# SarodYatawatta/smart-calibration

Hardware: AMD Instinct MI355X
Metric: env-steps/sec (whole node), elastic-net SAC (higher is better)
Workload: dtype fp32; 1 GPU; model=elasticnet-sac, N=20, M=20, input_dims=420, global_batch=64, replay=1024, reward_scale=20, prioritized=False, parallelism=dp1

## Files before the change

### setup.py

```python

import os
from pathlib import Path

from setuptools import setup

os.environ.setdefault("PYTORCH_ROCM_ARCH", "gfx950")

from torch.utils.cpp_extension import BuildExtension, CUDAExtension

ROOT = Path(__file__).resolve().parent
CSRC = ROOT / "smartcal_amd" / "ops" / "csrc"

sources = [str(CSRC / f) for f in [
    "bindings.hip",
    "fused_linear.hip",
    "gemm_f32.hip",
    "elementwise.hip",
    "enet_solver.hip",
    "als_sweep.hip",
    "conv2d.hip",
    "per.hip",
    "fused_linear_bf16.hip",
    "attention.hip",
    "cgemm.hip",
    "coherency.hip",
    "shapelet.hip",
    "beam.hip",
    "dft_image.hip",
    "hessianres.hip",
    "two_loop.hip",
    "gather_sum.hip",
]]

# ... 17 lines not shown
```

### smartcal_amd/envs/enet.py

```python

from __future__ import annotations

from typing import Optional

import numpy as np
import torch

from .. import gymapi
from ..gymapi import spaces
from ..ops import enet as enet_ops
from ..utils.device import default_device

LOW = 1e-3
HIGH = 1e-1


class ENetEnv(gymapi.Env):

    metadata = {"render.modes": ["human"]}

    def __init__(self, M: int = 5, N: int = 15, provide_hint: bool = False,
                 device: Optional[torch.device] = None):
        super().__init__()
        self.K = 2
# ... 20 lines not shown
        self._sample_problem()

    def _sample_problem(self):
        dev = self.device
        A = torch.randn(self.N, self.M, dtype=torch.float32, device=dev)
        self.A = A / torch.norm(A)
        self.Mo = int(torch.randint(3, self.M, (1,)).item())
        z0 = torch.randn(self.Mo, dtype=torch.float32, device=dev)
        self.x0 = torch.zeros(self.M, dtype=torch.float32, device=dev)
        self.x0[np.random.randint(0, self.M, self.Mo)] = z0
        self.y0 = self.A @ self.x0

    def _observe_y(self):
        n = torch.randn(self.N, dtype=torch.float32, device=self.device)
        self.y = self.y0 + self.SNR * torch.norm(self.y0) / torch.norm(n) * n

    def reset(self):
        self._sample_problem()
        self.hint = None
        self.rho = LOW * torch.ones(self.K, dtype=torch.float32)
        observation = {
            "A": self.A.reshape(-1),
            "eig": torch.zeros(self.N, dtype=torch.float32,
                               device=self.device),
        }
        return observation

    def step(self, action, keepnoise: bool = False):
        done = False
        if not torch.is_tensor(action):
            action = torch.as_tensor(np.asarray(action).reshape(-1),
                                     dtype=torch.float32)
        action = action.detach().reshape(-1)
        action = torch.nan_to_num(action, nan=0.0, posinf=1.0, neginf=-1.0)

        if self.device.type == "cuda" and action.device == self.device:
            scaled = action * (HIGH - LOW) / 2 + (HIGH + LOW) / 2
            penalty = -0.1 * ((scaled < LOW).sum() + (scaled > HIGH).sum())
            rho = scaled.clamp(LOW, HIGH)
            self.rho = rho
            if not keepnoise or self.y is None:
                self._observe_y()
            x, EE, reward = enet_ops.solve_and_influence_device(
                self.A, self.y, rho, penalty.to(torch.float32))
            self.x = x
            EE = torch.nan_to_num(EE, nan=0.0, posinf=1e6, neginf=-1e6)
            reward = torch.nan_to_num(reward, nan=-100.0, posinf=1e6,
                                      neginf=-1e6)
            observation = {"A": self.A.reshape(-1), "eig": EE}
            info: dict = {}
            if self.provide_hint:
                if self.hint is None:
                    self.hint = self.get_hint()
                return observation, reward, done, self.hint, info
            return observation, reward, done, info

        action = action.to("cpu", torch.float32)
        self.rho = action * (HIGH - LOW) / 2 + (HIGH + LOW) / 2
        penalty = 0.0
        for ci in range(self.K):
            if self.rho[ci] < LOW:
                self.rho[ci] = LOW
                penalty += -0.1
            if self.rho[ci] > HIGH:
                self.rho[ci] = HIGH
                penalty += -0.1

        if not keepnoise or self.y is None:
            self._observe_y()

        x, EE, reward = enet_ops.solve_and_influence(
# ... 65 lines not shown
                if mse < best[1]:
                    best = ((l1, l2), mse)
        hint_ = np.array(best[0], dtype=np.float64)
        return (hint_ - (HIGH + LOW) / 2) / ((HIGH - LOW) / 2)

    def close(self):
        pass


def obs_to_state(observation) -> torch.Tensor:
    if not isinstance(observation, dict):
        if torch.is_tensor(observation):
            return observation.reshape(-1).to(torch.float32)
        return torch.as_tensor(np.asarray(observation),
                               dtype=torch.float32).reshape(-1)
    eig = observation["eig"]
    A = observation["A"]
    if not torch.is_tensor(eig):
        eig = torch.as_tensor(eig, dtype=torch.float32)
    if not torch.is_tensor(A):
        A = torch.as_tensor(A, dtype=torch.float32)
    return torch.cat((eig.reshape(-1), A.reshape(-1).to(eig.device)))

try:
    from sklearn.base import BaseEstimator as _SKBase
except Exception:
    _SKBase = object


class SKEnet(_SKBase):
# ... 23 lines not shown
```

### smartcal_amd/envs/vec_enet.py

```python

from __future__ import annotations

from typing import Optional

import numpy as np
import torch

from ..ops import enet as enet_ops
from ..utils.device import default_device
from .enet import HIGH, LOW


class VecENetEnv:

    def __init__(self, E: int, M: int = 5, N: int = 15,
                 reward_clamp: Optional[float] = None,
                 device: Optional[torch.device] = None):
        self.E = int(E)
        self.M = int(M)
        self.N = int(N)
        self.K = 2
        self.reward_clamp = reward_clamp
        self.device = device if device is not None else default_device()
        self.SNR = 0.1
# ... 24 lines not shown
        self._sample_problems()
        self.y = None
        return {"A": self.A.reshape(self.E, -1),
                "eig": torch.zeros(self.E, self.N, dtype=torch.float32,
                                   device=self.device)}

    def step(self, actions, keepnoise: bool = False):
        if torch.is_tensor(actions):
            a = actions.detach().to(dtype=torch.float32) \
                .reshape(self.E, self.K)
        else:
            a = torch.as_tensor(np.asarray(actions), dtype=torch.float32) \
                .reshape(self.E, self.K)
        if a.device != self.device:
            a = a.to(self.device)
        a = torch.nan_to_num(a.detach(), nan=0.0, posinf=1.0, neginf=-1.0)
        scaled = a * (HIGH - LOW) / 2 + (HIGH + LOW) / 2
        penalty = -0.1 * ((scaled < LOW).sum(1)
                          + (scaled > HIGH).sum(1)).to(torch.float32)
        rho = scaled.clamp(LOW, HIGH)
        self.rho = rho
        if not keepnoise or self.y is None:
            self._observe_y()
        x, EE, reward = enet_ops.solve_and_influence_batch(
            self.A, self.y, rho, penalty)
        self.x = x
        EE = torch.nan_to_num(EE, nan=0.0, posinf=1e6, neginf=-1e6)
        reward = torch.nan_to_num(reward, nan=-100.0, posinf=1e6,
                                  neginf=-1e6)
        if self.reward_clamp is not None:
            reward = reward.clamp(-self.reward_clamp, self.reward_clamp)
        obs = {"A": self.A.reshape(self.E, -1), "eig": EE}
        done = torch.zeros(self.E, dtype=torch.bool, device=self.device)
        return obs, reward, done, {}

    def solution_error(self) -> torch.Tensor:
        return ((self.x0 - self.x).norm(dim=1)
                / self.x0.norm(dim=1).clamp(min=1e-12))
```

### smartcal_amd/ops/csrc/bindings.hip

```cpp

#include <ATen/hip/HIPContext.h>
#include <c10/hip/HIPStream.h>
#include <torch/extension.h>

#include <algorithm>
#include <tuple>

#include "common.h"

#define HMAX 7

extern "C" __global__ void fused_linear_fwd_kernel(
    const float*, const float*, const float*, const float*, const float*,
    float*, float*, float*, int, int, int, int, int);
extern "C" __global__ void ln_act_bwd_kernel(const float*, const float*,
                                             const float*, const float*,
                                             const float*, float*, float*,
                                             float*, int, int, int, int,
                                             int);
extern "C" __global__ void gemm_f32_nn_kernel(const float*, const float*,
                                              float*, int, int, int);
extern "C" __global__ void gemm_f32_tn_kernel(const float*, const float*,
                                              float*, float*, int, int, int,
                                              int);
// ... 16 lines not shown
extern "C" __global__ void conv2d_k5s2_fwd_kernel(
    const float*, const float*, const float*, float*, int, int, int, int,
    int, int, int);
extern "C" __global__ void conv2d_k5s2_dx_kernel(
    const float*, const float*, float*, int, int, int, int, int, int, int);
extern "C" __global__ void conv2d_k5s2_dw_kernel(
    const float*, const float*, float*, float*, int, int, int, int, int,
    int, int);
struct c32b { float x, y; };
extern "C" __global__ void als_sweep_kernel(
    const c32b*, const c32b*, const c32b*, const int*, const int*,
    const int*, c32b*, c32b*, int, int, int, int, int, int);
extern "C" __global__ void enet_influence_kernel(
    const float*, const float*, const float*, const float*, const float*,
    const int*, const float*, const float*, float*, float*, int, int, int);
extern "C" __global__ void per_sample_kernel(const float*, const float*,
                                             long*, float*, float*, int, int,
                                             float);
extern "C" __global__ void fused_linear_bf16_fwd_kernel(
    const float*, const float*, const float*, const float*, const float*,
    float*, float*, float*, int, int, int, int, int);
extern "C" __global__ void gemm_bf16_nn_kernel(const float*, const float*,
                                               float*, int, int, int);
extern "C" __global__ void gemm_bf16_tn_kernel(const float*, const float*,
                                               float*, int, int, int, int);
extern "C" __global__ void attn_fwd_kernel(const float*, const float*,
                                           const float*, float*, float*,
                                           int, int, int);
extern "C" __global__ void attn_bwd_kernel(const float*, const float*,
                                           const float*, const float*,
// ... 607 lines not shown
                     (int)history);
  return {x, Y, S, nh};
}

std::tuple<at::Tensor, at::Tensor> enet_influence(
    const at::Tensor& A, const at::Tensor& y, const at::Tensor& x,
    const at::Tensor& Y, const at::Tensor& S, const at::Tensor& nh,
    const at::Tensor& penalty, const at::Tensor& rho) {
  check_f32(A, "A");
  check_f32(rho, "rho");
  const int E = A.size(0), N = A.size(1), M = A.size(2);
  TORCH_CHECK(N <= 32 && M <= 32, "enet influence supports N,M <= 32");
  TORCH_CHECK(rho.numel() == 2 * E, "rho must be (E, 2)");
  auto EE = at::empty({E, N}, A.options());
  auto reward = at::empty({E}, A.options());
  const int lds_floats = N * M + M * N + N * N + 2 * HMAX * M + HMAX * N + N
                         + M + N + HMAX;
  hipLaunchKernelGGL(enet_influence_kernel, dim3(E), dim3(64),
                     lds_floats * sizeof(float), stream(),
                     A.data_ptr<float>(), y.data_ptr<float>(),
                     x.data_ptr<float>(), Y.data_ptr<float>(),
                     S.data_ptr<float>(), nh.data_ptr<int>(),
                     penalty.data_ptr<float>(), rho.data_ptr<float>(),
                     EE.data_ptr<float>(), reward.data_ptr<float>(),
                     E, N, M);
  return {EE, reward};
}

#define PER_LDS_MAX_N 32768
#define PER_MAX_B 4096

std::tuple<at::Tensor, at::Tensor, at::Tensor> per_sample(
    const at::Tensor& priorities, const at::Tensor& u, double beta) {
  check_f32(priorities, "priorities");
  check_f32(u, "u");
  const int n = priorities.numel();
  const int B = u.numel();
  TORCH_CHECK(n >= 1 && n <= PER_LDS_MAX_N,
              "per_sample: n must be in [1, 32768]");
  TORCH_CHECK(B >= 1 && B <= PER_MAX_B, "per_sample: B must be in [1, 4096]");
  auto idx = at::empty({B}, priorities.options().dtype(at::kLong));
// ... 392 lines not shown
  m.def("fused_linear_bwd_dz_into", &fused_linear_bwd_dz_into);
  m.def("mlp_chain_fwd", &mlp_chain_fwd, py::arg("x"), py::arg("Ws"),
        py::arg("bs"), py::arg("gammas"), py::arg("betas"), py::arg("acts"),
        py::arg("bf16") = false, py::arg("save") = true);
  m.def("critic_fwd", &critic_fwd, py::arg("state"), py::arg("action"),
        py::arg("Ws"), py::arg("bs"), py::arg("gammas"), py::arg("betas"),
        py::arg("acts"), py::arg("save") = true);
  m.def("als_sweep", &als_sweep);
  m.def("conv2d_k5s2_fwd", &conv2d_k5s2_fwd);
  m.def("conv2d_k5s2_bwd", &conv2d_k5s2_bwd);
  m.def("tanh_gauss_fwd", &tanh_gauss_fwd);
  m.def("tanh_gauss_bwd", &tanh_gauss_bwd);
  m.def("fused_adam", &fused_adam);
  m.def("enet_lbfgs_solve", &enet_lbfgs_solve);
  m.def("enet_influence", &enet_influence);
  m.def("per_sample", &per_sample);
  m.def("per_update", &per_update);
  m.def("fused_linear_bf16_fwd", &fused_linear_bf16_fwd);
  m.def("mfma_gemm_nn_bf16", &mfma_gemm_nn_bf16);
  m.def("mfma_gemm_tn_bias_into_bf16", &mfma_gemm_tn_bias_into_bf16);
  m.def("attn_fwd", &attn_fwd);
  m.def("attn_bwd", &attn_bwd);
  m.def("cgemm_nn_bcast", &cgemm_nn_bcast);
  m.def("coherency_predict", &coherency_predict);
  m.def("shapelet_predict", &shapelet_predict, py::arg("C"),
        py::arg("uvw_scaled"), py::arg("hdr"), py::arg("coff"),
        py::arg("coef"), py::arg("clk"), py::arg("soff"), py::arg("fdelta"),
        py::arg("E") = py::none(), py::arg("p") = py::none(),
        py::arg("q") = py::none(), py::arg("sbase") = 0);
  m.def("station_beam", &station_beam);
// ... 9 lines not shown
```

### smartcal_amd/ops/csrc/enet_solver.hip

```cpp

#include "common.h"

#define HMAX 7
#define TOL_GRAD 1e-7f
#define TOL_CHANGE 1e-9f
#define NMAX 32

struct LdsLayout {
  float* __restrict__ A;
  float* __restrict__ y;
  float* __restrict__ x;
  float* __restrict__ g;
  float* __restrict__ gprev;
  float* __restrict__ d;
  float* __restrict__ x0;
  float* __restrict__ r;
  float* __restrict__ S;
  float* __restrict__ Yh;
  float* __restrict__ bg0;
  float* __restrict__ bg1;
  float* __restrict__ ro;
  float* __restrict__ al;
  float* __restrict__ xprev;
};
// ... 200 lines not shown
  }

  if (!done) {
    t = br_t[low];
    f_new = br_f[low];
    if (lane < M) {
      L.g[lane] = br_g[low][lane];
      float xd = t * L.d[lane];
      L.x[lane] = L.x0[lane] + (isfinite(xd) ? xd : 0.f);
    }
  }
  *t_io = t;
  return f_new;
}

extern "C" __global__ __launch_bounds__(64) void enet_lbfgs_solve_kernel(
    const float* __restrict__ Ag,
    const float* __restrict__ yg,
    const float* __restrict__ rhog,
    float* __restrict__ xg,
    float* __restrict__ Yg,
    float* __restrict__ Sg,
    int* __restrict__ nhistg,
    int E, int N, int M, int epochs, int max_iter, int history) {
  extern __shared__ float smem[];
  const int env = blockIdx.x;
  const int lane = threadIdx.x;
  if (history > HMAX) history = HMAX;

  LdsLayout L;
  float* p = smem;
  L.A = p; p += N * M;
  L.y = p; p += N;
  L.x = p; p += M;
  L.g = p; p += M;
  L.gprev = p; p += M;
  L.d = p; p += M;
  L.x0 = p; p += M;
  L.r = p; p += N;
  L.S = p; p += HMAX * M;
  L.Yh = p; p += HMAX * M;
  L.bg0 = p; p += M;
  L.bg1 = p; p += M;
  L.ro = p; p += HMAX;
  L.al = p; p += HMAX;
  L.xprev = p; p += M;

  for (int i = lane; i < N * M; i += WAVE) L.A[i] = Ag[(long)env * N * M + i];
  __builtin_amdgcn_s_barrier();
  RegA Ar;
#pragma unroll
  for (int j = 0; j < 32; ++j)
    Ar.row[j] = (lane < N && j < M) ? L.A[lane * M + j] : 0.f;
#pragma unroll
  for (int i = 0; i < 32; ++i)
    Ar.col[i] = (lane < M && i < N) ? L.A[i * M + lane] : 0.f;
  if (lane < N) L.y[lane] = yg[(long)env * N + lane];
  if (lane < M) {
    L.x[lane] = 0.f;
    L.d[lane] = 0.f;
    L.gprev[lane] = 0.f;
  }
  const float rho1 = rhog[env * 2 + 0];
  const float rho2 = rhog[env * 2 + 1];

  int nhist = 0;
  int n_iter = 0;
  float t = 1.f, H_diag = 1.f, prev_loss = 0.f;
  float prev_epoch_loss = 1e30f;
  if (lane < M) L.xprev[lane] = 1e30f;

  for (int epoch = 0; epoch < epochs; ++epoch) {
    float loss = eval_loss_grad(L, Ar, N, M, rho1, rho2);
    if (fabsf(loss - prev_epoch_loss) <= 3e-7f * fmaxf(1.f, fabsf(loss)))
      break;
    prev_epoch_loss = loss;
    {
      float dx = (lane < M) ? fabsf(L.x[lane] - L.xprev[lane]) : 0.f;
      float dmax = wave_max(dx);
// ... 73 lines not shown
      loss = strong_wolfe(L, Ar, N, M, rho1, rho2, loss, gtd, &t);
      if (!isfinite(loss)) {
        if (lane < M) L.x[lane] = L.x0[lane];
        loss = eval_loss_grad(L, Ar, N, M, rho1, rho2);
        outer_done = true;
        break;
      }

      if (lds_absmax(L.g, M) <= TOL_GRAD) { outer_done = true; break; }
      float step_max = lds_absmax(L.d, M) * fabsf(t);
      if (step_max <= TOL_CHANGE) break;
      if (fabsf(loss - prev_loss) < TOL_CHANGE) break;
    }
    if (outer_done) break;
  }

  if (lane < M) xg[(long)env * M + lane] = L.x[lane];
  for (int h = 0; h < HMAX; ++h) {
    if (lane < M) {
      float yv = (h < nhist) ? L.Yh[h * M + lane] : 0.f;
      float sv = (h < nhist) ? L.S[h * M + lane] : 0.f;
      Yg[((long)env * HMAX + h) * M + lane] = yv;
      Sg[((long)env * HMAX + h) * M + lane] = sv;
    }
  }
  if (lane == 0) nhistg[env] = nhist;
}

extern "C" __global__ __launch_bounds__(64) void enet_influence_kernel(
    const float* __restrict__ Ag,
    const float* __restrict__ yg,
    const float* __restrict__ xg,
    const float* __restrict__ Yg,
    const float* __restrict__ Sg,
    const int* __restrict__ nhistg,
    const float* __restrict__ peng,
    const float* __restrict__ rhog,
    float* __restrict__ EEg,
    float* __restrict__ rewardg,
    int E, int N, int M) {
  extern __shared__ float smem[];
  const int env = blockIdx.x;
  const int lane = threadIdx.x;
  const int nh = nhistg[env];

  float* p = smem;
  float* A = p; p += N * M;
  float* Q = p; p += M * N;
  float* B = p; p += N * N;
  float* Sv = p; p += HMAX * M;
  float* Yv = p; p += HMAX * M;
  float* alv = p; p += HMAX * N;
  float* ev = p; p += N;
  float* xs = p; p += M;
  float* ys_ = p; p += N;
  float* ro = p; p += HMAX;

  for (int i = lane; i < N * M; i += WAVE) A[i] = Ag[(long)env * N * M + i];
  for (int i = lane; i < HMAX * M; i += WAVE) {
    Sv[i] = Sg[(long)env * HMAX * M + i];
    Yv[i] = Yg[(long)env * HMAX * M + i];
  }
  if (lane < M) xs[lane] = xg[(long)env * M + lane];
  if (lane < N) ys_[lane] = yg[(long)env * N + lane];

  __builtin_amdgcn_s_barrier();
  float qc[32];
#pragma unroll
  for (int m = 0; m < 32; ++m)
    qc[m] = (lane < N && m < M) ? -2.f * A[lane * M + m] : 0.f;

  const float rho1f = rhog[env * 2];
  const float lo = fmaxf(1e-6f, rho1f);
  const float hi = 8.f * (1.f + rho1f) * (1.f + rho1f);
  float ys = 1.f, yy = 1.f;
  for (int i = 0; i < nh; ++i) {
    float ysi = lds_dot(&Yv[i * M], &Sv[i * M], M);
    float ssi = lds_dot(&Sv[i * M], &Sv[i * M], M);
    float yyi = lds_dot(&Yv[i * M], &Yv[i * M], M);
    float r = (ysi > lo * ssi && yyi < hi * ssi) ? 1.f / ysi : 0.f;
    if (lane == 0) ro[i] = r;
    if (r != 0.f) {
      ys = ysi;
      yy = yyi;
    }
  }
  __builtin_amdgcn_s_barrier();
// ... 90 lines not shown
  const float ee_floor = 1.f - 1.f / fmaxf(rho1f, 1e-6f);
  if (lane < N) ev[lane] = fmaxf(B[lane * N + lane] + 1.f, ee_floor);

  for (int phase = 0; phase < N; ++phase) {
    int start = phase & 1;
    int i0 = start + 2 * lane;
    float a0 = 0.f, a1 = 0.f;
    bool act = (i0 + 1 < N);
    if (act) { a0 = ev[i0]; a1 = ev[i0 + 1]; }
    if (act && a0 > a1) {
      ev[i0] = a1;
      ev[i0 + 1] = a0;
    }
  }

  if (lane < N) EEg[(long)env * N + lane] = ev[lane];

  float ri = 0.f, yl = 0.f;
  if (lane < N) {
    float ax = 0.f;
    for (int m = 0; m < M; ++m) ax += A[lane * M + m] * xs[m];
    ri = ax - ys_[lane];
    yl = ys_[lane];
  }
  float err = sqrtf(wave_sum(ri * ri));
  float ynorm = sqrtf(wave_sum(yl * yl));
  float emin = ev[0], emax = ev[N - 1];
  if (lane == 0)
    rewardg[env] = ynorm / err + emin / emax + peng[env];
}
```

### smartcal_amd/ops/enet.py

```python

from __future__ import annotations

from typing import Tuple

import torch

from . import ext


def lbfgs_solve_reference(A: torch.Tensor, y: torch.Tensor,
                          rho1: float, rho2: float,
                          epochs: int = 20, max_iter: int = 10,
                          history: int = 7):
    from ..optim import LBFGSNew

    x = torch.zeros(A.shape[1], requires_grad=True, device=A.device)
    opt = LBFGSNew([x], history_size=history, max_iter=max_iter,
                   line_search_fn=True, batch_mode=False)

    def closure():
        if torch.is_grad_enabled():
            opt.zero_grad()
        err = y - A @ x
        loss = (err * err).sum() + rho1 * (x * x).sum() + rho2 * x.abs().sum()
# ... 40 lines not shown
                               rho: torch.Tensor, penalty: torch.Tensor,
                               epochs: int = 20, max_iter: int = 10,
                               history: int = 7):
    ext()
    Ab = A.unsqueeze(0).contiguous()
    yb = y.unsqueeze(0).contiguous()
    rho2d = rho.reshape(1, 2).contiguous()
    x, Yc, Sc, nh = ext().enet_lbfgs_solve(Ab, yb, rho2d,
                                           epochs, max_iter, history)
    EE, reward = ext().enet_influence(Ab, yb, x, Yc, Sc, nh,
                                      penalty.reshape(1).contiguous(),
                                      rho2d)
    return x[0], EE[0], reward[0]


def solve_and_influence(A: torch.Tensor, y: torch.Tensor,
                        rho1, rho2, penalty: float,
                        epochs: int = 20, max_iter: int = 10,
                        history: int = 7):
    from . import use_hip

    if use_hip(A):
        Ab = A.unsqueeze(0).contiguous()
        yb = y.unsqueeze(0).contiguous()
        rho = torch.tensor([[float(rho1), float(rho2)]], device=A.device)
        x, Yc, Sc, nh = ext().enet_lbfgs_solve(Ab, yb, rho, epochs,
                                               max_iter, history)
        pen = torch.tensor([penalty], device=A.device)
        EE, reward = ext().enet_influence(Ab, yb, x, Yc, Sc, nh, pen, rho)
        return x[0], EE[0], reward[0]
# ... 35 lines not shown
```

### smartcal_amd/rl/buffers.py

```python

from __future__ import annotations

import pickle
from typing import Optional, Tuple

import numpy as np
import torch

from ..ops import per as per_ops


class ReplayBuffer:

    def __init__(self, max_size: int, input_dims, n_actions: int,
                 device: Optional[torch.device] = None):
        self.mem_size = int(max_size)
        self.mem_cntr = 0
        self.device = device if device is not None else torch.device("cpu")
        dims = list(input_dims) if not isinstance(input_dims, int) \
            else [input_dims]
        self.state_memory = torch.zeros((self.mem_size, *dims),
                                        dtype=torch.float32,
                                        device=self.device)
        self.new_state_memory = torch.zeros_like(self.state_memory)
# ... 6 lines not shown
                                           device=self.device)
        self.hint_memory = torch.zeros((self.mem_size, n_actions),
                                       dtype=torch.float32,
                                       device=self.device)
        self.filename = "replaymem_sac.model"

    def __len__(self):
        return min(self.mem_cntr, self.mem_size)

    def _as(self, x, like: torch.Tensor):
        if torch.is_tensor(x):
            return x.detach().to(like.device, like.dtype).reshape(like.shape)
        return torch.as_tensor(np.asarray(x), dtype=like.dtype,
                               device=like.device).reshape(like.shape)

    def store_transition(self, state, action, reward, state_, done,
                         hint=None):
        i = self.mem_cntr % self.mem_size
        self.state_memory[i] = self._as(state, self.state_memory[i])
        self.new_state_memory[i] = self._as(state_, self.new_state_memory[i])
        self.action_memory[i] = self._as(action, self.action_memory[i])
        if torch.is_tensor(reward):
            self.reward_memory[i] = reward.detach().to(
                self.reward_memory.device, torch.float32).reshape(())
        else:
            self.reward_memory[i] = float(reward)
        self.terminal_memory[i] = bool(done)
        if hint is not None:
            self.hint_memory[i] = self._as(hint, self.hint_memory[i])
        self.mem_cntr += 1

    def store_batch(self, states, actions, rewards, states_, dones,
                    hints=None):
# ... 159 lines not shown
```

### smartcal_amd/rl/sac.py

```python

from __future__ import annotations

import os
from typing import Optional

import numpy as np
import torch
import torch.nn.functional as F

from ..envs.enet import obs_to_state
from ..utils.device import default_device
from ..utils.flatten import FlatParams, FusedAdam
from .buffers import PERBuffer, ReplayBuffer
from .networks import CriticMLP, SACActorMLP


class Agent:
    def __init__(self, gamma, lr_a, lr_c, input_dims, batch_size, n_actions,
                 max_mem_size=100, tau=0.001, reward_scale=2, alpha=0.1,
                 name_prefix="", prioritized=False, use_hint=False,
                 device: Optional[torch.device] = None,
                 checkpoint_dir="./", learn_alpha=False,
                 grad_hook=None):
        self.gamma = gamma
# ... 192 lines not shown
    def enable_cuda_graph(self):
        assert not self.use_hint and not self.prioritized
        assert self.device.type == "cuda"
        B = self.batch_size
        mem = self.replaymem
        self._g_idx = torch.zeros(B, dtype=torch.long, device=self.device)
        self._g_state = torch.zeros(B, mem.state_memory.shape[1],
                                    device=self.device)
        self._g_new_state = torch.zeros_like(self._g_state)
        self._g_action = torch.zeros(B, self.n_actions, device=self.device)
        self._g_reward = torch.zeros(B, 1, device=self.device)
        self._g_done = torch.zeros(B, 1, dtype=torch.bool,
                                   device=self.device)
        self._g_hint = torch.zeros(B, self.n_actions, device=self.device)

        n = len(mem)
        if n > 0:
            torch.randint(0, n, (B,), device=self.device, out=self._g_idx)
            torch.index_select(mem.state_memory, 0, self._g_idx,
                               out=self._g_state)
            torch.index_select(mem.new_state_memory, 0, self._g_idx,
                               out=self._g_new_state)
            torch.index_select(mem.action_memory, 0, self._g_idx,
                               out=self._g_action)
            torch.index_select(mem.reward_memory, 0, self._g_idx,
                               out=self._g_reward.view(-1))
            self._g_reward.mul_(self.scale)
            torch.index_select(mem.terminal_memory, 0, self._g_idx,
                               out=self._g_done.view(-1))

        torch.cuda.synchronize()
        s = torch.cuda.Stream()
        s.wait_stream(torch.cuda.current_stream())
        with torch.cuda.stream(s):
            for _ in range(3):
                self._learn_body(self._g_state, self._g_new_state,
                                 self._g_action, self._g_reward,
                                 self._g_done, self._g_hint)
        torch.cuda.current_stream().wait_stream(s)
        torch.cuda.synchronize()

        g = torch.cuda.CUDAGraph()
        with torch.cuda.graph(g):
            self._learn_body(self._g_state, self._g_new_state,
                             self._g_action, self._g_reward,
                             self._g_done, self._g_hint)
        self._graph = g

    def disable_cuda_graph(self):
        self._graph = None

    def _learn_graphed(self):
        mem = self.replaymem
        n = len(mem)
        torch.randint(0, n, (self.batch_size,), device=self.device,
                      out=self._g_idx)
        torch.index_select(mem.state_memory, 0, self._g_idx,
                           out=self._g_state)
        torch.index_select(mem.new_state_memory, 0, self._g_idx,
                           out=self._g_new_state)
        torch.index_select(mem.action_memory, 0, self._g_idx,
                           out=self._g_action)
        torch.index_select(mem.reward_memory, 0, self._g_idx,
                           out=self._g_reward.view(-1))
        self._g_reward.mul_(self.scale)
        torch.index_select(mem.terminal_memory, 0, self._g_idx,
                           out=self._g_done.view(-1))
        self._graph.replay()
        self.learn_counter += 1

    def learn(self):
        if self.replaymem.mem_cntr < self.batch_size:
            return

        if getattr(self, "_graph", None) is not None:
            return self._learn_graphed()

        if self.prioritized:
            (state, action, reward, new_state, done, hint), idxs, is_w = \
                self.replaymem.sample_buffer(self.batch_size)
            is_w = is_w.to(self.device).unsqueeze(1)
        else:
# ... 85 lines not shown
```

Before: 458.6 env-steps/s.

## Fuse env step, replay store and replay gather into custom HIP kernels

Replaces the many small PyTorch ops in the ENet environment step (action scaling, penalty, noise observation, nan_to_num, observation concat) with prologue and epilogue kernels around the existing solver. The epilogue writes a flat state buffer, so state flattening needs no copy. Replay-buffer stores and the six-op batch gather are each replaced by a single kernel, and the noise-norm scale is cached per problem. The goal is to cut kernel launch and Python overhead per env step, at the cost of more custom code paths and some changed nan handling semantics.

Result: slower. 408.4 env-steps/s (-10.9%).

```diff
diff --git a/setup.py b/setup.py
--- a/setup.py
+++ b/setup.py
@@ -17,6 +17,7 @@
     "gemm_f32.hip",
     "elementwise.hip",
     "enet_solver.hip",
+    "replay.hip",
     "als_sweep.hip",
     "conv2d.hip",
     "per.hip",
diff --git a/smartcal_amd/envs/enet.py b/smartcal_amd/envs/enet.py
--- a/smartcal_amd/envs/enet.py
+++ b/smartcal_amd/envs/enet.py
@@ -58,6 +58,13 @@
     def _observe_y(self):
         n = torch.randn(self.N, dtype=torch.float32, device=self.device)
         self.y = self.y0 + self.SNR * torch.norm(self.y0) / torch.norm(n) * n
+
+    def _noise_scale(self):
+        key = getattr(self, "_noise_scale_key", None)
+        if key is None or key[0] is not self.y0 or key[1] != self.SNR:
+            self._noise_scale_val = self.SNR * torch.norm(self.y0)
+            self._noise_scale_key = (self.y0, self.SNR)
+        return self._noise_scale_val
 
     def reset(self):
         self._sample_problem()
@@ -76,22 +83,26 @@
             action = torch.as_tensor(np.asarray(action).reshape(-1),
                                      dtype=torch.float32)
         action = action.detach().reshape(-1)
-        action = torch.nan_to_num(action, nan=0.0, posinf=1.0, neginf=-1.0)
 
         if self.device.type == "cuda" and action.device == self.device:
-            scaled = action * (HIGH - LOW) / 2 + (HIGH + LOW) / 2
-            penalty = -0.1 * ((scaled < LOW).sum() + (scaled > HIGH).sum())
-            rho = scaled.clamp(LOW, HIGH)
-            self.rho = rho
+            A = self.A.unsqueeze(0).contiguous()
+            a = action.to(torch.float32).reshape(1, self.K).contiguous()
             if not keepnoise or self.y is None:
-                self._observe_y()
-            x, EE, reward = enet_ops.solve_and_influence_device(
-                self.A, self.y, rho, penalty.to(torch.float32))
-            self.x = x
-            EE = torch.nan_to_num(EE, nan=0.0, posinf=1e6, neginf=-1e6)
-            reward = torch.nan_to_num(reward, nan=-100.0, posinf=1e6,
-                                      neginf=-1e6)
-            observation = {"A": self.A.reshape(-1), "eig": EE}
+                n = torch.randn(self.N, dtype=torch.float32,
+                                device=self.device)
+                rho, y, x, reward, flat = enet_ops.env_step_fused(
+                    A, a, LOW, HIGH, y0=self.y0.reshape(1, -1).contiguous(),
+                    noise=n.reshape(1, -1),
+                    s=self._noise_scale().reshape(1),
+                    nrm=torch.norm(n).reshape(1))
+            else:
+                rho, y, x, reward, flat = enet_ops.env_step_fused(
+                    A, a, LOW, HIGH, y=self.y.reshape(1, -1).contiguous())
+            self.rho = rho[0]
+            self.y = y[0]
+            self.x = x[0]
+            reward = reward[0]
+            observation = enet_ops.FlatObs(flat[0], self.N)
             info: dict = {}
             if self.provide_hint:
                 if self.hint is None:
@@ -99,6 +110,7 @@
                 return observation, reward, done, self.hint, info
             return observation, reward, done, info
 
+        action = torch.nan_to_num(action, nan=0.0, posinf=1.0, neginf=-1.0)
         action = action.to("cpu", torch.float32)
         self.rho = action * (HIGH - LOW) / 2 + (HIGH + LOW) / 2
         penalty = 0.0
@@ -194,6 +206,10 @@
             return observation.reshape(-1).to(torch.float32)
         return torch.as_tensor(np.asarray(observation),
                                dtype=torch.float32).reshape(-1)
+    if isinstance(observation, enet_ops.FlatObs):
+        flat = observation.flat_state()
+        if flat is not None:
+            return flat
     eig = observation["eig"]
     A = observation["A"]
     if not torch.is_tensor(eig):
diff --git a/smartcal_amd/envs/vec_enet.py b/smartcal_amd/envs/vec_enet.py
--- a/smartcal_amd/envs/vec_enet.py
+++ b/smartcal_amd/envs/vec_enet.py
@@ -62,6 +62,8 @@
                 .reshape(self.E, self.K)
         if a.device != self.device:
             a = a.to(self.device)
+        if self.device.type == "cuda":
+            return self._step_fused(a.detach(), keepnoise)
         a = torch.nan_to_num(a.detach(), nan=0.0, posinf=1.0, neginf=-1.0)
         scaled = a * (HIGH - LOW) / 2 + (HIGH + LOW) / 2
         penalty = -0.1 * ((scaled < LOW).sum(1)
@@ -82,6 +84,27 @@
         done = torch.zeros(self.E, dtype=torch.bool, device=self.device)
         return obs, reward, done, {}
 
+    def _step_fused(self, a, keepnoise: bool):
+        if not keepnoise or self.y is None:
+            n = torch.randn(self.E, self.N, dtype=torch.float32,
+                            device=self.device)
+            if getattr(self, "_noise_scale_y0", None) is not self.y0:
+                self._noise_scale = self.SNR * self.y0.norm(dim=1)
+                self._noise_scale_y0 = self.y0
+            rho, y, x, reward, flat = enet_ops.env_step_fused(
+                self.A.contiguous(), a.contiguous(), LOW, HIGH,
+                y0=self.y0.contiguous(), noise=n, s=self._noise_scale,
+                nrm=n.norm(dim=1), nrm_floor=1e-12,
+                reward_clamp=self.reward_clamp)
+        else:
+            rho, y, x, reward, flat = enet_ops.env_step_fused(
+                self.A.contiguous(), a.contiguous(), LOW, HIGH,
+                y=self.y.contiguous(), reward_clamp=self.reward_clamp)
+        self.rho, self.y, self.x = rho, y, x
+        obs = enet_ops.FlatObs(flat, self.N)
+        done = torch.zeros(self.E, dtype=torch.bool, device=self.device)
+        return obs, reward, done, {}
+
     def solution_error(self) -> torch.Tensor:
         return ((self.x0 - self.x).norm(dim=1)
                 / self.x0.norm(dim=1).clamp(min=1e-12))
diff --git a/smartcal_amd/ops/csrc/bindings.hip b/smartcal_amd/ops/csrc/bindings.hip
--- a/smartcal_amd/ops/csrc/bindings.hip
+++ b/smartcal_amd/ops/csrc/bindings.hip
@@ -54,6 +54,20 @@
 extern "C" __global__ void enet_influence_kernel(
     const float*, const float*, const float*, const float*, const float*,
     const int*, const float*, const float*, float*, float*, int, int, int);
+extern "C" __global__ void enet_step_prologue_kernel(
+    const float*, const float*, const float*, const float*, const float*,
+    float*, float*, float*, int, int, float, float, float, float, float, int);
+extern "C" __global__ void enet_step_epilogue_kernel(
+    const float*, const float*, float*, float*, int, int, int, float, int);
+struct HintVals { float v[8]; };
+extern "C" __global__ void replay_store_kernel(
+    const float*, const float*, const float*, const float*, const float*,
+    float*, float*, float*, float*, unsigned char*, float*, HintVals, float,
+    int, int, int, int, long);
+extern "C" __global__ void replay_gather_kernel(
+    const long*, const float*, const float*, const float*, const float*,
+    const unsigned char*, float*, float*, float*, float*, unsigned char*,
+    float, int, int, long);
 extern "C" __global__ void per_sample_kernel(const float*, const float*,
                                              long*, float*, float*, int, int,
                                              float);
@@ -691,8 +705,7 @@
   TORCH_CHECK(rho.numel() == 2 * E, "rho must be (E, 2)");
   auto EE = at::empty({E, N}, A.options());
   auto reward = at::empty({E}, A.options());
-  const int lds_floats = N * M + M * N + N * N + 2 * HMAX * M + HMAX * N + N
-                         + M + N + HMAX;
+  const int lds_floats = N * M + N * N + 2 * HMAX * M + N + M + N + HMAX;
   hipLaunchKernelGGL(enet_influence_kernel, dim3(E), dim3(64),
                      lds_floats * sizeof(float), stream(),
                      A.data_ptr<float>(), y.data_ptr<float>(),
@@ -702,6 +715,160 @@
                      EE.data_ptr<float>(), reward.data_ptr<float>(),
                      E, N, M);
   return {EE, reward};
+}
+
+std::tuple<at::Tensor, at::Tensor, at::Tensor, at::Tensor, at::Tensor>
+enet_step(const at::Tensor& A, const at::Tensor& action, const at::Tensor& y0,
+          const at::Tensor& noise, const at::Tensor& s, const at::Tensor& nrm,
+          double c1, double c2, double low, double high, double nrm_floor,
+          bool y_ready, c10::optional<double> reward_clamp, int64_t epochs,
+          int64_t max_iter, int64_t history) {
+  check_f32(A, "A");
+  check_f32(action, "action");
+  check_f32(y0, "y0");
+  TORCH_CHECK(A.dim() == 3, "A must be (E, N, M)");
+  const int E = A.size(0), N = A.size(1), M = A.size(2);
+  TORCH_CHECK(E >= 1 && N >= 1 && M >= 1 && N <= 32 && M <= 32,
+              "enet step supports 1 <= N,M <= 32");
+  TORCH_CHECK(action.numel() == 2L * E, "action must be (E, 2)");
+  TORCH_CHECK(y0.numel() == (long)E * N, "y0 must be (E, N)");
+  if (!y_ready) {
+    check_f32(noise, "noise");
+    check_f32(s, "s");
+    check_f32(nrm, "nrm");
+    TORCH_CHECK(noise.numel() == (long)E * N, "noise must be (E, N)");
+    TORCH_CHECK(s.numel() == E && nrm.numel() == E, "s, nrm must be (E,)");
+  }
+  auto rho = at::empty({E, 2}, A.options());
+  auto pen = at::empty({E}, A.options());
+  auto y = at::empty({E, N}, A.options());
+  hipLaunchKernelGGL(enet_step_prologue_kernel, dim3(E), dim3(64), 0,
+                     stream(), action.data_ptr<float>(),
+                     y0.data_ptr<float>(), noise.data_ptr<float>(),
+                     s.data_ptr<float>(), nrm.data_ptr<float>(),
+                     rho.data_ptr<float>(), pen.data_ptr<float>(),
+                     y.data_ptr<float>(), E, N, (float)c1, (float)c2,
+                     (float)low, (float)high, (float)nrm_floor,
+                     y_ready ? 1 : 0);
+  auto [x, Yc, Sc, nh] = enet_lbfgs_solve(A, y, rho, epochs, max_iter,
+                                          history);
+  auto [EE, reward] = enet_influence(A, y, x, Yc, Sc, nh, pen, rho);
+  auto state = at::empty({E, (long)N + (long)N * M}, A.options());
+  hipLaunchKernelGGL(enet_step_epilogue_kernel, dim3(E), dim3(64), 0,
+                     stream(), A.data_ptr<float>(), EE.data_ptr<float>(),
+                     reward.data_ptr<float>(), state.data_ptr<float>(), E, N,
+                     M, reward_clamp ? (float)*reward_clamp : 0.f,
+                     reward_clamp ? 1 : 0);
+  return {rho, y, x, reward, state};
+}
+
+void replay_store(at::Tensor& state_mem, at::Tensor& new_state_mem,
+                  at::Tensor& action_mem, at::Tensor& reward_mem,
+                  at::Tensor& terminal_mem, at::Tensor& hint_mem,
+                  int64_t slot, const at::Tensor& state,
+                  const at::Tensor& state_, const at::Tensor& action,
+                  const c10::optional<at::Tensor>& reward, double reward_val,
+                  bool done, const c10::optional<at::Tensor>& hint,
+                  const std::vector<double>& hint_vals) {
+  check_f32(state_mem, "state_mem");
+  check_f32(new_state_mem, "new_state_mem");
+  check_f32(action_mem, "action_mem");
+  check_f32(reward_mem, "reward_mem");
+  check_f32(hint_mem, "hint_mem");
+  check_f32(state, "state");
+  check_f32(state_, "state_");
+  check_f32(action, "action");
+  TORCH_CHECK(terminal_mem.is_cuda() && terminal_mem.is_contiguous()
+              && terminal_mem.scalar_type() == at::kBool, "terminal_mem");
+  const long cap = state_mem.size(0);
+  TORCH_CHECK(cap >= 1 && slot >= 0 && slot < cap, "slot out of range");
+  const long D = state_mem.numel() / cap, nA = action_mem.numel() / cap;
+  TORCH_CHECK(new_state_mem.numel() == cap * D && reward_mem.numel() == cap
+              && terminal_mem.numel() == cap && hint_mem.numel() == cap * nA,
+              "replay memories disagree in size");
+  TORCH_CHECK(state.numel() == D && state_.numel() == D
+              && action.numel() == nA, "transition does not fit the slot");
+  TORCH_CHECK(D >= 1 && nA >= 1 && D < (1L << 30) && nA < (1L << 30),
+              "row too wide");
+  const float* rptr = nullptr;
+  if (reward) {
+    check_f32(*reward, "reward");
+    TORCH_CHECK(reward->numel() == 1, "reward must be a scalar");
+    rptr = reward->data_ptr<float>();
+  }
+  int mode = 0;
+  const float* hptr = nullptr;
+  HintVals hv = {};
+  if (hint) {
+    check_f32(*hint, "hint");
+    TORCH_CHECK(hint->numel() == nA, "hint size");
+    hptr = hint->data_ptr<float>();
+    mode = 2;
+  } else if (!hint_vals.empty()) {
+    TORCH_CHECK((long)hint_vals.size() == nA && nA <= 8,
+                "by-value hint needs n_actions <= 8 values");
+    for (long k = 0; k < nA; ++k) hv.v[k] = (float)hint_vals[k];
+    mode = 1;
+  }
+  const int threads = 256;
+  const int blocks = (int)((std::max(D, nA) + threads - 1) / threads);
+  hipLaunchKernelGGL(replay_store_kernel, dim3(blocks), dim3(threads), 0,
+                     stream(), state.data_ptr<float>(),
+                     state_.data_ptr<float>(), action.data_ptr<float>(), rptr,
+                     hptr, state_mem.data_ptr<float>(),
+                     new_state_mem.data_ptr<float>(),
+                     action_mem.data_ptr<float>(),
+                     reward_mem.data_ptr<float>(),
+                     (unsigned char*)terminal_mem.data_ptr<bool>(),
+                     hint_mem.data_ptr<float>(), hv, (float)reward_val,
+                     done ? 1 : 0, mode, (int)D, (int)nA, (long)slot);
+}
+
+void replay_gather(const at::Tensor& idx, int64_t n,
+                   const at::Tensor& state_mem,
+                   const at::Tensor& new_state_mem,
+                   const at::Tensor& action_mem, const at::Tensor& reward_mem,
+                   const at::Tensor& terminal_mem, at::Tensor& g_state,
+                   at::Tensor& g_new_state, at::Tensor& g_action,
+                   at::Tensor& g_reward, at::Tensor& g_done, double scale) {
+  check_f32(state_mem, "state_mem");
+  check_f32(new_state_mem, "new_state_mem");
+  check_f32(action_mem, "action_mem");
+  check_f32(reward_mem, "reward_mem");
+  check_f32(g_state, "g_state");
+  check_f32(g_new_state, "g_new_state");
+  check_f32(g_action, "g_action");
+  check_f32(g_reward, "g_reward");
+  TORCH_CHECK(idx.is_cuda() && idx.is_contiguous()
+              && idx.scalar_type() == at::kLong, "idx must be int64 on GPU");
+  TORCH_CHECK(terminal_mem.is_cuda() && terminal_mem.is_contiguous()
+              && terminal_mem.scalar_type() == at::kBool, "terminal_mem");
+  TORCH_CHECK(g_done.is_cuda() && g_done.is_contiguous()
+              && g_done.scalar_type() == at::kBool, "g_done");
+  const long cap = state_mem.size(0), B = idx.numel();
+  TORCH_CHECK(cap >= 1 && n >= 1 && n <= cap, "n must be in 1..capacity");
+  TORCH_CHECK(B >= 1, "empty batch");
+  const long D = state_mem.numel() / cap, nA = action_mem.numel() / cap;
+  TORCH_CHECK(new_state_mem.numel() == cap * D && reward_mem.numel() == cap
+              && terminal_mem.numel() == cap,
+              "replay memories disagree in size");
+  TORCH_CHECK(g_state.numel() == B * D && g_new_state.numel() == B * D
+              && g_action.numel() == B * nA && g_reward.numel() == B
+              && g_done.numel() == B, "batch buffers do not fit");
+  TORCH_CHECK(D >= 1 && nA >= 1 && D < (1L << 30) && nA < (1L << 30),
+              "row too wide");
+  hipLaunchKernelGGL(replay_gather_kernel, dim3((unsigned)B), dim3(256), 0,
+                     stream(), (const long*)idx.data_ptr<int64_t>(),
+                     state_mem.data_ptr<float>(),
+                     new_state_mem.data_ptr<float>(),
+                     action_mem.data_ptr<float>(),
+                     reward_mem.data_ptr<float>(),
+                     (const unsigned char*)terminal_mem.data_ptr<bool>(),
+                     g_state.data_ptr<float>(),
+                     g_new_state.data_ptr<float>(),
+                     g_action.data_ptr<float>(), g_reward.data_ptr<float>(),
+                     (unsigned char*)g_done.data_ptr<bool>(), (float)scale,
+                     (int)D, (int)nA, (long)n);
 }
 
 #define PER_LDS_MAX_N 32768
@@ -1124,6 +1291,13 @@
   m.def("fused_adam", &fused_adam);
   m.def("enet_lbfgs_solve", &enet_lbfgs_solve);
   m.def("enet_influence", &enet_influence);
+  m.def("enet_step", &enet_step, py::arg("A"), py::arg("action"),
+        py::arg("y0"), py::arg("noise"), py::arg("s"), py::arg("nrm"),
+        py::arg("c1"), py::arg("c2"), py::arg("low"), py::arg("high"),
+        py::arg("nrm_floor"), py::arg("y_ready"), py::arg("reward_clamp"),
+        py::arg("epochs"), py::arg("max_iter"), py::arg("history"));
+  m.def("replay_store", &replay_store);
+  m.def("replay_gather", &replay_gather);
   m.def("per_sample", &per_sample);
   m.def("per_update", &per_update);
   m.def("fused_linear_bf16_fwd", &fused_linear_bf16_fwd);
diff --git a/smartcal_amd/ops/csrc/enet_solver.hip b/smartcal_amd/ops/csrc/enet_solver.hip
--- a/smartcal_amd/ops/csrc/enet_solver.hip
+++ b/smartcal_amd/ops/csrc/enet_solver.hip
@@ -238,22 +238,9 @@
   return f_new;
 }
 
-extern "C" __global__ __launch_bounds__(64) void enet_lbfgs_solve_kernel(
-    const float* __restrict__ Ag,
-    const float* __restrict__ yg,
-    const float* __restrict__ rhog,
-    float* __restrict__ xg,
-    float* __restrict__ Yg,
-    float* __restrict__ Sg,
-    int* __restrict__ nhistg,
-    int E, int N, int M, int epochs, int max_iter, int history) {
-  extern __shared__ float smem[];
-  const int env = blockIdx.x;
-  const int lane = threadIdx.x;
-  if (history > HMAX) history = HMAX;
-
-  LdsLayout L;
-  float* p = smem;
+__device__ __forceinline__ static float* carve_solve_lds(LdsLayout& L,
+                                                         float* p, int N,
+                                                         int M) {
   L.A = p; p += N * M;
   L.y = p; p += N;
   L.x = p; p += M;
@@ -269,9 +256,14 @@
   L.ro = p; p += HMAX;
   L.al = p; p += HMAX;
   L.xprev = p; p += M;
-
-  for (int i = lane; i < N * M; i += WAVE) L.A[i] = Ag[(long)env * N * M + i];
-  __builtin_amdgcn_s_barrier();
+  return p;
+}
+
+__device__ __forceinline__ static int enet_solve_body(
+    const LdsLayout& L, int N, int M, float rho1, float rho2, int epochs,
+    int max_iter, int history) {
+  const int lane = threadIdx.x;
+  if (history > HMAX) history = HMAX;
   RegA Ar;
 #pragma unroll
   for (int j = 0; j < 32; ++j)
@@ -279,14 +271,11 @@
 #pragma unroll
   for (int i = 0; i < 32; ++i)
     Ar.col[i] = (lane < M && i < N) ? L.A[i * M + lane] : 0.f;
-  if (lane < N) L.y[lane] = yg[(long)env * N + lane];
   if (lane < M) {
     L.x[lane] = 0.f;
     L.d[lane] = 0.f;
     L.gprev[lane] = 0.f;
   }
-  const float rho1 = rhog[env * 2 + 0];
-  const float rho2 = rhog[env * 2 + 1];
 
   int nhist = 0;
   int n_iter = 0;
@@ -390,6 +379,33 @@
     }
     if (outer_done) break;
   }
+  return nhist;
+}
+
+extern "C" __global__ __launch_bounds__(64) void enet_lbfgs_solve_kernel(
+    const float* __restrict__ Ag,
+    const float* __restrict__ yg,
+    const float* __restrict__ rhog,
+    float* __restrict__ xg,
+    float* __restrict__ Yg,
+    float* __restrict__ Sg,
+    int* __restrict__ nhistg,
+    int E, int N, int M, int epochs, int max_iter, int history) {
+  extern __shared__ float smem[];
+  const int env = blockIdx.x;
+  const int lane = threadIdx.x;
+
+  LdsLayout L;
+  carve_solve_lds(L, smem, N, M);
+
+  for (int i = lane; i < N * M; i += WAVE) L.A[i] = Ag[(long)env * N * M + i];
+  if (lane < N) L.y[lane] = yg[(long)env * N + lane];
+  __builtin_amdgcn_s_barrier();
+  const float rho1 = rhog[env * 2 + 0];
+  const float rho2 = rhog[env * 2 + 1];
+
+  const int nhist = enet_solve_body(L, N, M, rho1, rho2, epochs, max_iter,
+                                    history);
 
   if (lane < M) xg[(long)env * M + lane] = L.x[lane];
   for (int h = 0; h < HMAX; ++h) {
@@ -403,50 +419,17 @@
   if (lane == 0) nhistg[env] = nhist;
 }
 
-extern "C" __global__ __launch_bounds__(64) void enet_influence_kernel(
-    const float* __restrict__ Ag,
-    const float* __restrict__ yg,
-    const float* __restrict__ xg,
-    const float* __restrict__ Yg,
-    const float* __restrict__ Sg,
-    const int* __restrict__ nhistg,
-    const float* __restrict__ peng,
-    const float* __restrict__ rhog,
-    float* __restrict__ EEg,
-    float* __restrict__ rewardg,
-    int E, int N, int M) {
-  extern __shared__ float smem[];
-  const int env = blockIdx.x;
-  const int lane = threadIdx.x;
-  const int nh = nhistg[env];
-
-  float* p = smem;
-  float* A = p; p += N * M;
-  float* Q = p; p += M * N;
-  float* B = p; p += N * N;
-  float* Sv = p; p += HMAX * M;
-  float* Yv = p; p += HMAX * M;
-  float* alv = p; p += HMAX * N;
-  float* ev = p; p += N;
-  float* xs = p; p += M;
-  float* ys_ = p; p += N;
-  float* ro = p; p += HMAX;
-
-  for (int i = lane; i < N * M; i += WAVE) A[i] = Ag[(long)env * N * M + i];
-  for (int i = lane; i < HMAX * M; i += WAVE) {
-    Sv[i] = Sg[(long)env * HMAX * M + i];
-    Yv[i] = Yg[(long)env * HMAX * M + i];
-  }
-  if (lane < M) xs[lane] = xg[(long)env * M + lane];
-  if (lane < N) ys_[lane] = yg[(long)env * N + lane];
-
-  __builtin_amdgcn_s_barrier();
+__device__ __forceinline__ static float enet_influence_body(
+    const float* A, const float* Sv, const float* Yv, const float* xs,
+    const float* ys_, float* B, float* ev, float* ro, int nh, float rho1f,
+    float pen, int N, int M) {
+  const int lane = threadIdx.x;
+
   float qc[32];
 #pragma unroll
   for (int m = 0; m < 32; ++m)
     qc[m] = (lane < N && m < M) ? -2.f * A[lane * M + m] : 0.f;
 
-  const float rho1f = rhog[env * 2];
   const float lo = fmaxf(1e-6f, rho1f);
   const float hi = 8.f * (1.f + rho1f) * (1.f + rho1f);
   float ys = 1.f, yy = 1.f;
@@ -567,8 +550,6 @@
     }
   }
 
-  if (lane < N) EEg[(long)env * N + lane] = ev[lane];
-
   float ri = 0.f, yl = 0.f;
   if (lane < N) {
     float ax = 0.f;
@@ -579,6 +560,127 @@
   float err = sqrtf(wave_sum(ri * ri));
   float ynorm = sqrtf(wave_sum(yl * yl));
   float emin = ev[0], emax = ev[N - 1];
-  if (lane == 0)
-    rewardg[env] = ynorm / err + emin / emax + peng[env];
-}
+  return ynorm / err + emin / emax + pen;
+}
+
+extern "C" __global__ __launch_bounds__(64) void enet_influence_kernel(
+    const float* __restrict__ Ag,
+    const float* __restrict__ yg,
+    const float* __restrict__ xg,
+    const float* __restrict__ Yg,
+    const float* __restrict__ Sg,
+    const int* __restrict__ nhistg,
+    const float* __restrict__ peng,
+    const float* __restrict__ rhog,
+    float* __restrict__ EEg,
+    float* __restrict__ rewardg,
+    int E, int N, int M) {
+  extern __shared__ float smem[];
+  const int env = blockIdx.x;
+  const int lane = threadIdx.x;
+  const int nh = nhistg[env];
+
+  float* p = smem;
+  float* A = p; p += N * M;
+  float* B = p; p += N * N;
+  float* Sv = p; p += HMAX * M;
+  float* Yv = p; p += HMAX * M;
+  float* ev = p; p += N;
+  float* xs = p; p += M;
+  float* ys_ = p; p += N;
+  float* ro = p; p += HMAX;
+
+  for (int i = lane; i < N * M; i += WAVE) A[i] = Ag[(long)env * N * M + i];
+  for (int i = lane; i < HMAX * M; i += WAVE) {
+    Sv[i] = Sg[(long)env * HMAX * M + i];
+    Yv[i] = Yg[(long)env * HMAX * M + i];
+  }
+  if (lane < M) xs[lane] = xg[(long)env * M + lane];
+  if (lane < N) ys_[lane] = yg[(long)env * N + lane];
+  __builtin_amdgcn_s_barrier();
+
+  const float reward = enet_influence_body(A, Sv, Yv, xs, ys_, B, ev, ro, nh,
+                                           rhog[env * 2], peng[env], N, M);
+  if (lane < N) EEg[(long)env * N + lane] = ev[lane];
+  if (lane == 0) rewardg[env] = reward;
+}
+
+__device__ __forceinline__ static float nan_to_num_f(float v, float nanv,
+                                                     float posv, float negv) {
+  if (isnan(v)) return nanv;
+  if (isinf(v)) return v > 0.f ? posv : negv;
+  return v;
+}
+
+__device__ __forceinline__ static float mul_rn(float a, float b) {
+#pragma clang fp contract(off)
+  return a * b;
+}
+
+__device__ __forceinline__ static float add_rn(float a, float b) {
+#pragma clang fp contract(off)
+  return a + b;
+}
+
+__device__ __forceinline__ static float div_rn(float a, float b) {
+#pragma clang fp contract(off)
+  return a / b;
+}
+
+extern "C" __global__ __launch_bounds__(64) void enet_step_prologue_kernel(
+    const float* __restrict__ actg,
+    const float* __restrict__ y0g,
+    const float* __restrict__ noiseg,
+    const float* __restrict__ sg,
+    const float* __restrict__ nrmg,
+    float* __restrict__ rhog,
+    float* __restrict__ peng,
+    float* __restrict__ yg,
+    int E, int N, float c1, float c2, float low, float high,
+    float nrm_floor, int y_ready) {
+  const int env = blockIdx.x;
+  const int lane = threadIdx.x;
+
+  float rho[2];
+  int nout = 0;
+#pragma unroll
+  for (int k = 0; k < 2; ++k) {
+    const float a = nan_to_num_f(actg[env * 2 + k], 0.f, 1.f, -1.f);
+    const float scaled = add_rn(mul_rn(mul_rn(a, c1), 0.5f), c2);
+    nout += (scaled < low) + (scaled > high);
+    rho[k] = fminf(fmaxf(scaled, low), high);
+  }
+  if (lane < 2) rhog[env * 2 + lane] = lane == 0 ? rho[0] : rho[1];
+  if (lane == 0) peng[env] = mul_rn(-0.1f, (float)nout);
+
+  if (lane < N) {
+    float yv = y0g[(long)env * N + lane];
+    if (!y_ready) {
+      float nrm = nrmg[env];
+      if (nrm < nrm_floor) nrm = nrm_floor;
+      const float t = div_rn(sg[env], nrm);
+      yv = add_rn(yv, mul_rn(t, noiseg[(long)env * N + lane]));
+    }
+    yg[(long)env * N + lane] = yv;
+  }
+}
+
+extern "C" __global__ __launch_bounds__(64) void enet_step_epilogue_kernel(
+    const float* __restrict__ Ag,
+    const float* __restrict__ EEg,
+    float* __restrict__ rewardg,
+    float* __restrict__ stateg,
+    int E, int N, int M, float reward_clamp, int has_clamp) {
+  const int env = blockIdx.x;
+  const int lane = threadIdx.x;
+  if (lane == 0) {
+    float reward = nan_to_num_f(rewardg[env], -100.f, 1e6f, -1e6f);
+    if (has_clamp) reward = fminf(fmaxf(reward, -reward_clamp), reward_clamp);
+    rewardg[env] = reward;
+  }
+  float* st = stateg + (long)env * (N + N * M);
+  if (lane < N)
+    st[lane] = nan_to_num_f(EEg[(long)env * N + lane], 0.f, 1e6f, -1e6f);
+  for (int i = lane; i < N * M; i += WAVE)
+    st[N + i] = Ag[(long)env * N * M + i];
+}
diff --git a/smartcal_amd/ops/csrc/replay.hip b/smartcal_amd/ops/csrc/replay.hip
--- /dev/null
+++ b/smartcal_amd/ops/csrc/replay.hip
@@ -0,0 +1,64 @@
+
+#include "common.h"
+
+struct HintVals {
+  float v[8];
+};
+
+#define HINT_NONE 0
+#define HINT_BY_VALUE 1
+#define HINT_POINTER 2
+
+extern "C" __global__ void replay_store_kernel(
+    const float* __restrict__ state, const float* __restrict__ state_,
+    const float* __restrict__ action, const float* __restrict__ reward_ptr,
+    const float* __restrict__ hint_ptr, float* __restrict__ state_mem,
+    float* __restrict__ new_state_mem, float* __restrict__ action_mem,
+    float* __restrict__ reward_mem, unsigned char* __restrict__ terminal_mem,
+    float* __restrict__ hint_mem, HintVals hint_vals, float reward_val,
+    int done, int hint_mode, int D, int nA, long slot) {
+  const int i = blockIdx.x * blockDim.x + threadIdx.x;
+  if (i < D) {
+    state_mem[slot * D + i] = state[i];
+    new_state_mem[slot * D + i] = state_[i];
+  }
+  if (i < nA) {
+    action_mem[slot * nA + i] = action[i];
+    if (hint_mode == HINT_BY_VALUE) {
+      float h = hint_vals.v[0];
+#pragma unroll
+      for (int k = 1; k < 8; ++k) h = (i == k) ? hint_vals.v[k] : h;
+      hint_mem[slot * nA + i] = h;
+    } else if (hint_mode == HINT_POINTER) {
+      hint_mem[slot * nA + i] = hint_ptr[i];
+    }
+  }
+  if (i == 0) {
+    reward_mem[slot] = reward_ptr ? reward_ptr[0] : reward_val;
+    terminal_mem[slot] = done ? 1 : 0;
+  }
+}
+
+extern "C" __global__ void replay_gather_kernel(
+    const long* __restrict__ idx, const float* __restrict__ state_mem,
+    const float* __restrict__ new_state_mem,
+    const float* __restrict__ action_mem,
+    const float* __restrict__ reward_mem,
+    const unsigned char* __restrict__ terminal_mem,
+    float* __restrict__ g_state, float* __restrict__ g_new_state,
+    float* __restrict__ g_action, float* __restrict__ g_reward,
+    unsigned char* __restrict__ g_done, float scale, int D, int nA, long n) {
+  const long b = blockIdx.x;
+  long j = idx[b];
+  j = j < 0 ? 0 : (j >= n ? n - 1 : j);
+  for (int i = threadIdx.x; i < D; i += blockDim.x) {
+    g_state[b * D + i] = state_mem[j * D + i];
+    g_new_state[b * D + i] = new_state_mem[j * D + i];
+  }
+  for (int i = threadIdx.x; i < nA; i += blockDim.x)
+    g_action[b * nA + i] = action_mem[j * nA + i];
+  if (threadIdx.x == 0) {
+    g_reward[b] = reward_mem[j] * scale;
+    g_done[b] = terminal_mem[j];
+  }
+}
diff --git a/smartcal_amd/ops/enet.py b/smartcal_amd/ops/enet.py
--- a/smartcal_amd/ops/enet.py
+++ b/smartcal_amd/ops/enet.py
@@ -78,6 +78,44 @@
     return x[0], EE[0], reward[0]
 
 
+def env_step_fused(A: torch.Tensor, action: torch.Tensor, low: float,
+                   high: float, y0: torch.Tensor = None,
+                   noise: torch.Tensor = None, s: torch.Tensor = None,
+                   nrm: torch.Tensor = None, y: torch.Tensor = None,
+                   nrm_floor: float = 0.0, reward_clamp=None,
+                   epochs: int = 20, max_iter: int = 10, history: int = 7):
+    c1 = high - low
+    c2 = (high + low) / 2
+    if y is not None:
+        return ext().enet_step(A, action, y, y, y, y, c1, c2, low, high,
+                               0.0, True, reward_clamp, epochs, max_iter,
+                               history)
+    return ext().enet_step(A, action, y0, noise, s, nrm, c1, c2, low, high,
+                           nrm_floor, False, reward_clamp, epochs, max_iter,
+                           history)
+
+
+class FlatObs(dict):
+
+    def __init__(self, flat: torch.Tensor, n_eig: int):
+        super().__init__(eig=flat[..., :n_eig], A=flat[..., n_eig:])
+        self.flat = flat
+
+    def flat_state(self):
+        flat, eig, A = self.flat, self.get("eig"), self.get("A")
+        if (flat.dim() == 1 and flat.is_contiguous() and len(self) == 2
+                and torch.is_tensor(eig)
+                and torch.is_tensor(A) and eig.dim() == 1 and A.dim() == 1
+                and eig.dtype == flat.dtype == A.dtype == torch.float32
+                and eig.device == flat.device == A.device
+                and eig.stride(0) == 1 and A.stride(0) == 1
+                and eig.data_ptr() == flat.data_ptr()
+                and A.data_ptr() == flat.data_ptr() + 4 * eig.numel()
+                and eig.numel() + A.numel() == flat.numel()):
+            return flat
+        return None
+
+
 def solve_and_influence(A: torch.Tensor, y: torch.Tensor,
                         rho1, rho2, penalty: float,
                         epochs: int = 20, max_iter: int = 10,
diff --git a/smartcal_amd/rl/buffers.py b/smartcal_amd/rl/buffers.py
--- a/smartcal_amd/rl/buffers.py
+++ b/smartcal_amd/rl/buffers.py
@@ -44,9 +44,52 @@
         return torch.as_tensor(np.asarray(x), dtype=like.dtype,
                                device=like.device).reshape(like.shape)
 
+    def _dev_f32(self, x, numel: int) -> bool:
+        return (torch.is_tensor(x) and x.device == self.state_memory.device
+                and x.dtype == torch.float32 and x.numel() == numel
+                and x.is_contiguous())
+
+    def _store_kernel(self, i, state, action, reward, state_, done,
+                      hint) -> bool:
+        if not self.state_memory.is_cuda:
+            return False
+        D = self.state_memory.numel() // self.mem_size
+        nA = self.action_memory.shape[1]
+        if not (self._dev_f32(state, D) and self._dev_f32(state_, D)
+                and self._dev_f32(action, nA)):
+            return False
+        rew_t, rew_v = None, 0.0
+        if torch.is_tensor(reward):
+            if not self._dev_f32(reward, 1):
+                return False
+            rew_t = reward.detach()
+        else:
+            rew_v = float(reward)
+        hint_t, hint_v = None, []
+        if torch.is_tensor(hint) and hint.is_cuda:
+            if not self._dev_f32(hint, nA):
+                return False
+            hint_t = hint.detach()
+        elif hint is not None:
+            if nA > 8:
+                return False
+            hint_v = np.asarray(hint, dtype=np.float32).reshape(-1).tolist()
+            if len(hint_v) != nA:
+                return False
+        from ..ops import ext
+        ext().replay_store(self.state_memory, self.new_state_memory,
+                           self.action_memory, self.reward_memory,
+                           self.terminal_memory, self.hint_memory, i,
+                           state.detach(), state_.detach(), action.detach(),
+                           rew_t, rew_v, bool(done), hint_t, hint_v)
+        return True
+
     def store_transition(self, state, action, reward, state_, done,
                          hint=None):
         i = self.mem_cntr % self.mem_size
+        if self._store_kernel(i, state, action, reward, state_, done, hint):
+            self.mem_cntr += 1
+            return
         self.state_memory[i] = self._as(state, self.state_memory[i])
         self.new_state_memory[i] = self._as(state_, self.new_state_memory[i])
         self.action_memory[i] = self._as(action, self.action_memory[i])
diff --git a/smartcal_amd/rl/sac.py b/smartcal_amd/rl/sac.py
--- a/smartcal_amd/rl/sac.py
+++ b/smartcal_amd/rl/sac.py
@@ -230,20 +230,8 @@
                                    device=self.device)
         self._g_hint = torch.zeros(B, self.n_actions, device=self.device)
 
-        n = len(mem)
-        if n > 0:
-            torch.randint(0, n, (B,), device=self.device, out=self._g_idx)
-            torch.index_select(mem.state_memory, 0, self._g_idx,
-                               out=self._g_state)
-            torch.index_select(mem.new_state_memory, 0, self._g_idx,
-                               out=self._g_new_state)
-            torch.index_select(mem.action_memory, 0, self._g_idx,
-                               out=self._g_action)
-            torch.index_select(mem.reward_memory, 0, self._g_idx,
-                               out=self._g_reward.view(-1))
-            self._g_reward.mul_(self.scale)
-            torch.index_select(mem.terminal_memory, 0, self._g_idx,
-                               out=self._g_done.view(-1))
+        if len(mem) > 0:
+            self._gather_batch()
 
         torch.cuda.synchronize()
         s = torch.cuda.Stream()
@@ -266,22 +254,21 @@
     def disable_cuda_graph(self):
         self._graph = None
 
-    def _learn_graphed(self):
+    def _gather_batch(self):
+        from ..ops import ext
         mem = self.replaymem
         n = len(mem)
         torch.randint(0, n, (self.batch_size,), device=self.device,
                       out=self._g_idx)
-        torch.index_select(mem.state_memory, 0, self._g_idx,
-                           out=self._g_state)
-        torch.index_select(mem.new_state_memory, 0, self._g_idx,
-                           out=self._g_new_state)
-        torch.index_select(mem.action_memory, 0, self._g_idx,
-                           out=self._g_action)
-        torch.index_select(mem.reward_memory, 0, self._g_idx,
-                           out=self._g_reward.view(-1))
-        self._g_reward.mul_(self.scale)
-        torch.index_select(mem.terminal_memory, 0, self._g_idx,
-                           out=self._g_done.view(-1))
+        ext().replay_gather(self._g_idx, n, mem.state_memory,
+                            mem.new_state_memory, mem.action_memory,
+                            mem.reward_memory, mem.terminal_memory,
+                            self._g_state, self._g_new_state,
+                            self._g_action, self._g_reward, self._g_done,
+                            float(self.scale))
+
+    def _learn_graphed(self):
+        self._gather_batch()
         self._graph.replay()
         self.learn_counter += 1
 
```
